# skyhehe123/SA-SSD

Hardware: NVIDIA H100
Metric: KITTI frames/sec (~20k pts, car_cfg voxel grid) (higher is better)
Workload: dtype f32

## Files before the change

include/sassd_b200.h:

```cpp
#ifndef SASSD_B200_H
#define SASSD_B200_H

#include <stddef.h>
#include <stdint.h>

#ifdef __cplusplus
extern "C" {
#endif

typedef void* sassd_stream_t;

enum {
    SASSD_OK = 0,
    SASSD_ERR_ARG = -1,
    SASSD_ERR_LAUNCH = -2,
    SASSD_ERR_WORKSPACE = -3,
    SASSD_ERR_UNSUPPORTED = -4
};

enum {
    SASSD_FLAG_VOXEL_CAP = 1,
    SASSD_FLAG_ROWS_CAP = 2,
    SASSD_FLAG_GUIDED_CAP = 4,
    SASSD_FLAG_NMS_CAP = 8,
// ... 42 lines not shown
int sassd_anchor_mask(const int32_t* coors, const int32_t* d_rows, int rows_cap, int batch, int H, int W,
                      const int32_t* rects, int n_anchors, int threshold, uint8_t* mask,
                      void* ws, size_t ws_bytes, sassd_stream_t stream);

int sassd_hash_build(const int32_t* coors, const int32_t* d_rows, int rows_cap, int batch, int D, int H, int W,
                     int32_t* keys, int32_t* vals, int slots, int32_t* d_status, sassd_stream_t stream);
int sassd_rulebook_subm(const int32_t* coors, const int32_t* d_rows, int rows_cap, int D, int H, int W,
                        const int32_t* keys, const int32_t* vals, int slots, int32_t* nbr, int32_t* tile_mask,
                        sassd_stream_t stream);
size_t sassd_rulebook_conv_workspace_bytes(int batch, int Do, int Ho, int Wo);
int sassd_rulebook_conv_outputs(const int32_t* coors_in, const int32_t* d_rows_in, int rows_cap_in, int batch,
                                int D, int H, int W, int32_t* coors_out, int32_t* d_rows_out, int rows_cap_out,
                                int32_t* d_status, void* ws, size_t ws_bytes, sassd_stream_t stream);
int sassd_rulebook_conv_outputs_hash(const int32_t* coors_in, const int32_t* d_rows_in, int rows_cap_in, int batch,
                                     int D, int H, int W, int32_t* coors_out, int32_t* d_rows_out, int rows_cap_out,
                                     int32_t* keys_out, int32_t* vals_out, int slots_out, int32_t* d_status, void* ws,
                                     size_t ws_bytes, sassd_stream_t stream);
int sassd_rulebook_conv_nbr(const int32_t* coors_out, const int32_t* d_rows_out, int rows_cap_out, int D, int H, int W,
                            const int32_t* keys_in, const int32_t* vals_in, int slots_in, int32_t* nbr,
                            int32_t* tile_mask, sassd_stream_t stream);
int sassd_rulebook_pairs(const int32_t* nbr, const int32_t* d_rows_out, int rows_cap, int32_t* indice_pairs,
                         int32_t* indice_pair_num, sassd_stream_t stream);

enum { SASSD_GCONV_TABLE = 0, SASSD_GCONV_CONV2D = 1, SASSD_GCONV_ROWS = 2 };
enum { SASSD_PREC_FP32 = 0, SASSD_PREC_TF32X3 = 1, SASSD_PREC_F16X3 = 2 };
typedef struct {
    int32_t mode, precision;
    int32_t cin, cout, taps;
    int32_t in_stride, out_stride;
    int32_t rows_cap;
    int32_t batch, H, W;
    int32_t relu;
} sassd_gconv_desc;
int sassd_gconv(const sassd_gconv_desc* host_desc, const float* in, const float* weight, const float* scale,
                const float* shift, const int32_t* nbr, const int32_t* d_rows, float* out, sassd_stream_t stream);

size_t sassd_gconv_pack_bytes(int taps, int cin, int cout, int precision);
int sassd_gconv_pack(const float* weight, int taps, int cin, int cout, int precision, void* packed,
                     sassd_stream_t stream);

typedef struct {
    int32_t batch, H, W;
    int32_t cin, cin_stored;
    int32_t cout, taps, relu;
    int32_t out_f32_stride, out_split_ch;
    int32_t tile_order;
    int32_t n_split;
} sassd_conv2d_desc;
int sassd_conv2d_f16x3(const sassd_conv2d_desc* host_desc, const void* in_split, const void* wpack, const float* scale,
                       const float* shift, float* out_f32, void* out_split, sassd_stream_t stream);
#define SASSD_CONV2D_TILE_H 8
#define SASSD_CONV2D_TILE_W 16
#define SASSD_TILE_DIST_MAX 9
int sassd_conv2d_f16x3_occ(const sassd_conv2d_desc* host_desc, const void* in_split, const void* wpack,
                           const float* scale, const float* shift, float* out_f32, void* out_split,
                           const int32_t* tile_dist, int reach, const float* const_out, int32_t* counters,
                           sassd_stream_t stream);
int sassd_conv2d_f16x3_occ_bg(const sassd_conv2d_desc* host_desc, const void* in_split, const void* wpack,
                              const float* scale, const float* shift, float* out_f32, void* out_split,
                              const int32_t* tile_dist, int reach, const float* const_out, const void* bg_split,
                              const float* bg_f32, int32_t* counters, sassd_stream_t stream);
int sassd_sparse_to_bev_split(const float* feat, const int32_t* coors, const int32_t* d_rows, int rows_cap, int C,
                              int D, int H, int W, int batch, void* bev_split, int32_t* tile_dist,
                              sassd_stream_t stream);

typedef struct {
    int32_t cin, cout, taps;
    int32_t rows_cap, in_rows_cap;
    int32_t relu, out_ch, out_f32_stride;
} sassd_spconv_desc;
size_t sassd_spconv_pack_bytes(int taps, int cin_stored, int cout);
int sassd_spconv_pack(const float* weight, int taps, int cin, int cin_stored, int cout, void* packed,
                      sassd_stream_t stream);
#define SASSD_SPCONV_TILE_ROWS 128
size_t sassd_spconv_workspace_bytes(void);
int sassd_spconv_f16x3(const sassd_spconv_desc* host_desc, const void* in_split, const void* wpack, const float* scale,
                       const float* shift, const int32_t* nbr, const int32_t* tile_mask, const int32_t* d_rows,
                       void* out_split, float* out_f32, void* ws, size_t ws_bytes, int32_t* counters,
                       sassd_stream_t stream);
int sassd_features_to_split(const float* feat, const int32_t* d_rows, int rows_cap, int cin, int cs, void* out_split,
                            sassd_stream_t stream);
int sassd_split_rows_to_bev(const void* feat_split, const int32_t* coors, const int32_t* d_rows, int rows_cap, int C,
                            int D, int H, int W, int batch, void* bev_split, int32_t* tile_dist, sassd_stream_t stream);

int sassd_sparse_to_bev(const float* feat, const int32_t* coors, const int32_t* d_rows, int rows_cap, int C,
                        int D, int H, int W, float* bev, sassd_stream_t stream);

size_t sassd_decode_select_workspace_bytes(int batch, int n_anchors);
int sassd_decode_select(const float* head, int head_stride, int batch, int H, int W, int num_class,
                        const float* anchors, int anchors_per_frame, const uint8_t* mask, int n_anchors, float thr,
                        float* boxes, int32_t* labels, int32_t* index, int32_t* d_k, int k_cap,
                        int32_t* d_status, void* ws, size_t ws_bytes, sassd_stream_t stream);

int sassd_pswarp(const float* feat, int feat_stride, int batch, int H, int W, const float* boxes,
                 const int32_t* d_k, int k_cap, float off_x, float off_y, float spatial_scale,
                 float* scores, sassd_stream_t stream);

size_t sassd_rescore_nms_workspace_bytes(int batch, int k_cap, int nms_cap);
int sassd_rescore_nms(const float* boxes, const float* scores, const int32_t* labels, const int32_t* d_k,
                      int batch, int k_cap, float score_thr, float iou_thr, int nms_cap,
                      float* det, int32_t* d_ndet, int det_cap, int32_t* d_status,
                      void* ws, size_t ws_bytes, sassd_stream_t stream);

#define SASSD_KITTI_META 36
#define SASSD_KITTI_ROW 14
int sassd_kitti_format(const float* det, const int32_t* d_ndet, int batch, int det_cap, const double* meta,
                       double* rows, int32_t* n_out, sassd_stream_t stream);

typedef struct {
    const void* rows;
    int64_t plane_stride;
    int32_t row_stride;
    int32_t channels;
    int32_t split;
    int32_t pad;
} sassd_point_levels;

int sassd_three_nn(const float* mean, const int32_t* coors0, const int32_t* d_rows0, int rows_cap0,
                   const int32_t* coors1, const int32_t* d_rows1, const int32_t* coors2, const int32_t* d_rows2,
                   const int32_t* coors3, const int32_t* d_rows3, int32_t* idx, float* dist2, float* points_mean,
                   sassd_stream_t stream);
int sassd_point_aux_head(const int32_t* idx, const float* dist2, const int32_t* d_rows0, int rows_cap0,
                         const sassd_point_levels* host_levels, const float* w_fc_t, const float* w_out, float* cls,
                         float* reg, sassd_stream_t stream);

#define SASSD_GT_CAP_MAX 256
size_t sassd_loss_workspace_bytes(int batch, int gt_cap);
int sassd_points_in_boxes(const float* points_mean, const int32_t* d_rows, int rows_cap, const float* gt,
                          const int32_t* d_ngt, int batch, int gt_cap, int32_t* labels, float* offsets,
                          int32_t* d_npos, int32_t* d_status, sassd_stream_t stream);
int sassd_assign_rpn(const float* anchors, int anchors_per_frame, const uint8_t* mask, int n_anchors, int num_class,
                     const float* gt, const int32_t* gt_class, const int32_t* gt_label, const int32_t* d_ngt,
                     int batch, int gt_cap, const float* host_pos_thr, const float* host_neg_thr, int32_t* labels,
                     float* targets, float* ious, int32_t* d_npos, int32_t* d_status, void* ws, size_t ws_bytes,
                     sassd_stream_t stream);
int sassd_assign_pswarp(const float* gt, const int32_t* d_ngt, int batch, int gt_cap, const float* boxes, int n_box,
                        const int32_t* d_head, int head_cap, const int32_t* d_k, float pos_thr, float neg_thr,
                        int32_t* labels, float* ious, int32_t* d_npos, int32_t* d_status, void* ws,
                        size_t ws_bytes, sassd_stream_t stream);
int sassd_rpn_loss(const float* head, int head_stride, int batch, int H, int W, int num_class, const float* anchors,
                   int anchors_per_frame, int n_anchors, const int32_t* labels, const float* targets,
                   const int32_t* d_npos, float* out, void* ws, size_t ws_bytes, sassd_stream_t stream);
int sassd_pswarp_loss(const float* scores, const int32_t* labels, int batch, int n_box, const int32_t* d_npos,
                      float* out, void* ws, size_t ws_bytes, sassd_stream_t stream);
int sassd_aux_loss(const float* point_cls, const float* point_reg, const int32_t* labels, const float* offsets,
                   const int32_t* d_rows, int rows_cap, int batch, const int32_t* d_npos, float* out, void* ws,
                   size_t ws_bytes, sassd_stream_t stream);

size_t sassd_nms_workspace_bytes(int n);
int sassd_nms_mask(const float* boxes5, int n, float thr, uint64_t* mask, sassd_stream_t stream);
int sassd_nms_sorted(const float* boxes5, int n, float thr, int64_t* keep, int32_t* d_nkeep,
                     void* ws, size_t ws_bytes, sassd_stream_t stream);
int sassd_boxes_iou_bev(const float* boxes_a, int na, const float* boxes_b, int nb, float* iou, sassd_stream_t stream);

int sassd_rotate_overlap_eval(const float* boxes, const int32_t* box_off, const float* query, const int32_t* query_off,
                              const int64_t* out_off, int nframes, int criterion, int max_pairs_per_frame, float* out,
                              sassd_stream_t stream);
int sassd_kitti_match(int nframes, const double* overlaps, const int64_t* ov_off, const int32_t* gt_off,
                      const int32_t* dt_off, const int32_t* dc_off, const double* gt_alpha, const double* dt_alpha,
                      const double* dt_score, const double* dt_bbox, const double* dc_bbox, const int32_t* ign_gt,
                      const int32_t* ign_dt, int metric, double min_overlap, int compute_aos, int nthresh,
                      const double* thresholds, double* pr, double* tp_scores, int64_t* n_tp_scores);

#ifdef __cplusplus
}
#endif
// ... 2 lines not shown
```

sa-ssd_b200/csrc/spconv_split.cu:

```cuda
#include "tc_common.cuh"

namespace sps {

using namespace tc;

constexpr int BKC = 64;
constexpr int PROD_WARPS = 8;
constexpr int THREADS3 = CONS_THREADS + PROD_WARPS * 32;
constexpr int W_PROD = CONS_THREADS / 32;
constexpr int MAX_CTAS = 148;
constexpr int DEAL_MIN_GAIN = 14;

template <int BN>
struct Cfg3 {
    static constexpr int B_TILE_BYTES = BN * 128;
    static constexpr int STAGE_BYTES = 2 * A_TILE_BYTES + 2 * B_TILE_BYTES;
    static constexpr int STAGES = 4;
    static constexpr int NBR_TILE_BYTES = BM * 27 * 4;
    static constexpr int BAR_BYTES = 768;
    static constexpr int DEAL_INTS = MAX_CTAS + 1 + 33 + 2 + 1;
    static constexpr int SMEM_BYTES = STAGES * STAGE_BYTES + 2 * NBR_TILE_BYTES + 1024 + BAR_BYTES + DEAL_INTS * 4;
};

__device__ __forceinline__ void cp_async16(uint32_t dst, const void* src, uint32_t src_bytes) {
// ... 426 lines not shown

static size_t spconv_parts_bytes() { return (size_t)2 * sps::MAX_CTAS * sps::BM * 64 * sizeof(float); }

extern "C" size_t sassd_spconv_workspace_bytes(void) {
    return spconv_parts_bytes() + (size_t)sps::MAX_CTAS * 2 * sizeof(int32_t);
}

extern "C" int sassd_spconv_f16x3(const sassd_spconv_desc* d, const void* in_split, const void* wpack,
                                  const float* scale, const float* shift, const int32_t* nbr,
                                  const int32_t* tile_mask, const int32_t* d_rows, void* out_split, float* out_f32,
                                  void* ws, size_t ws_bytes, int32_t* counters, sassd_stream_t stream_) {
    if (!d || !in_split || !wpack || (!out_split && !out_f32)) return SASSD_ERR_ARG;
    if (d->cin < 8 || (d->cin & 7) || d->cin > 64 || d->cout < 1 || d->cout > 64 || d->taps < 1 || d->rows_cap < 0)
        return SASSD_ERR_ARG;
    if (d->taps > 1 && !nbr) return SASSD_ERR_ARG;
    if (tile_mask && d->taps > 27) return SASSD_ERR_ARG;
    if (out_split && ((d->out_ch & 7) || d->out_ch < d->cout)) return SASSD_ERR_ARG;
    if (out_f32 && (d->out_f32_stride & 3)) return SASSD_ERR_ARG;
    if (ws && ws_bytes < sassd_spconv_workspace_bytes()) return SASSD_ERR_WORKSPACE;
    if (d->rows_cap == 0) return SASSD_OK;
    sps::Args a;
    a.in = (const __half*)in_split; a.in_plane = (size_t)d->in_rows_cap * d->cin;
    a.wpack = wpack; a.scale = scale; a.shift = shift; a.nbr = nbr; a.tile_mask = tile_mask; a.d_rows = d_rows;
    a.out_split = (__half*)out_split; a.out_plane = (size_t)d->rows_cap * d->out_ch; a.out_f32 = out_f32;
    a.parts = (float*)ws;
    a.arrivals = ws ? (int*)((char*)ws + spconv_parts_bytes()) : nullptr;
    a.counters = counters;
    a.cin = d->cin; a.cout = d->cout; a.taps = d->taps; a.rows_cap = d->rows_cap; a.relu = d->relu;
    a.out_ch = d->out_ch; a.out_f32_stride = d->out_f32_stride;
    const int tiles = sassd_div_up(d->rows_cap, sps::BM), tpg = spconv_tpg(d->cin);
    if (d->taps == 1) return sps::dispatch3<0>(a, tiles, (cudaStream_t)stream_);
    return sps::dispatch3<1>(a, ws ? tiles * ((d->taps + tpg - 1) / tpg) : tiles, (cudaStream_t)stream_);
}

__global__ void features_to_split_kernel(const float* __restrict__ feat, const int* __restrict__ d_rows, int rows_cap,
                                         int cin, int cs, __half* __restrict__ out) {
    const int rows = d_rows ? min(*d_rows, rows_cap) : rows_cap;
    const long long total = (long long)rows * cs;
    const size_t plane = (size_t)rows_cap * cs;
    for (long long i = blockIdx.x * (long long)blockDim.x + threadIdx.x; i < total; i += (long long)gridDim.x * blockDim.x) {
        const int r = (int)(i / cs), c = (int)(i % cs);
        float hi = 0.f, lo = 0.f;
        if (c < cin) tc::split_f16(feat[(size_t)r * cin + c], hi, lo);
        out[i] = __float2half_rn(hi);
        out[i + plane] = __float2half_rn(lo);
    }
}

extern "C" int sassd_features_to_split(const float* feat, const int32_t* d_rows, int rows_cap, int cin, int cs,
                                       void* out_split, sassd_stream_t stream_) {
    if (!feat || !out_split || cin < 1 || cs < cin || (cs & 7)) return SASSD_ERR_ARG;
    if (rows_cap <= 0) return SASSD_OK;
    features_to_split_kernel<<<sassd_grid((long long)rows_cap * cs, 256), 256, 0, (cudaStream_t)stream_>>>(
        feat, d_rows, rows_cap, cin, cs, (__half*)out_split);
    return sassd_check_launch();
}

__global__ void split_rows_to_bev_kernel(const uint4* __restrict__ feat, size_t in_plane16, const int4* __restrict__ coors,
                                         const int* __restrict__ d_rows, int rows_cap, int C8, int D, int H, int W,
                                         size_t out_plane16, uint4* __restrict__ bev, int* __restrict__ tile_dist) {
    const int rows = min(*d_rows, rows_cap);
    const long long total = (long long)rows * C8;
    for (long long i = blockIdx.x * (long long)blockDim.x + threadIdx.x; i < total; i += (long long)gridDim.x * blockDim.x) {
        const int r = (int)(i / C8), q = (int)(i % C8);
        const int4 c = __ldg(&coors[r]);
        const size_t o = (((size_t)c.x * H + c.z) * W + c.w) * (size_t)(D * C8) + (size_t)c.y * C8 + q;
        bev[o] = __ldg(&feat[i]);
        bev[o + out_plane16] = __ldg(&feat[i + in_plane16]);
        if (tile_dist && q == 0) sassd_mark_conv2d_tiles(tile_dist, c.x, c.z, c.w, H, W);
    }
}

extern "C" int sassd_split_rows_to_bev(const void* feat_split, const int32_t* coors, const int32_t* d_rows, int rows_cap,
                                       int C, int D, int H, int W, int batch, void* bev_split, int32_t* tile_dist,
                                       sassd_stream_t stream_) {
    if (!feat_split || !coors || !d_rows || !bev_split || (C & 7) || batch < 1) return SASSD_ERR_ARG;
    if (rows_cap <= 0) return SASSD_OK;
    const size_t in_plane16 = (size_t)rows_cap * C / 8, out_plane16 = (size_t)batch * H * W * D * C / 8;
    split_rows_to_bev_kernel<<<sassd_grid((long long)rows_cap * (C / 8), 256), 256, 0, (cudaStream_t)stream_>>>(
        (const uint4*)feat_split, in_plane16, (const int4*)coors, d_rows, rows_cap, C / 8, D, H, W, out_plane16,
        (uint4*)bev_split, tile_dist);
    return sassd_check_launch();
}
```

sa-ssd_b200/lib.py:

```python
import ctypes
import os

from . import build as _build

c_int, c_float, c_size_t, c_void_p = ctypes.c_int, ctypes.c_float, ctypes.c_size_t, ctypes.c_void_p


class VoxelParams(ctypes.Structure):
    _fields_ = [("voxel_size", c_float * 3), ("range_min", c_float * 3), ("grid", ctypes.c_int32 * 3),
                ("max_points", ctypes.c_int32), ("max_voxels", ctypes.c_int32)]


class Conv2dDesc(ctypes.Structure):
    _fields_ = [(n, ctypes.c_int32) for n in ("batch", "H", "W", "cin", "cin_stored", "cout", "taps", "relu",
                                              "out_f32_stride", "out_split_ch", "tile_order", "n_split")]


class SpconvDesc(ctypes.Structure):
    _fields_ = [(n, ctypes.c_int32) for n in ("cin", "cout", "taps", "rows_cap", "in_rows_cap", "relu", "out_ch",
                                              "out_f32_stride")]


class GConvDesc(ctypes.Structure):
    _fields_ = [(n, ctypes.c_int32) for n in ("mode", "precision", "cin", "cout", "taps", "in_stride", "out_stride",
                                              "rows_cap", "batch", "H", "W", "relu")]


class PointLevels(ctypes.Structure):
    _fields_ = [("rows", c_void_p), ("plane_stride", ctypes.c_int64), ("row_stride", ctypes.c_int32),
                ("channels", ctypes.c_int32), ("split", ctypes.c_int32), ("pad", ctypes.c_int32)]


GCONV_TABLE, GCONV_CONV2D, GCONV_ROWS = 0, 1, 2
PREC_FP32, PREC_TF32X3, PREC_F16X3 = 0, 1, 2
CONV2D_TILE_H, CONV2D_TILE_W = 8, 16
TILE_DIST_MAX = 9
SPCONV_TILE_ROWS = 128
KITTI_META, KITTI_ROW = 36, 14
POINT_LEVEL_CHANNELS = (32, 64, 64)
POINT_FC_IN, POINT_FC_OUT = 160, 64
GT_CAP_MAX = 256

OK = 0
ERRORS = {-1: "SASSD_ERR_ARG", -2: "SASSD_ERR_LAUNCH", -3: "SASSD_ERR_WORKSPACE", -4: "SASSD_ERR_UNSUPPORTED"}
FLAGS = {1: "VOXEL_CAP", 2: "ROWS_CAP", 4: "GUIDED_CAP", 8: "NMS_CAP", 16: "HASH_FULL", 32: "DET_CAP",
         64: "GT_CAP", 128: "GATHER_CAP"}
GATHER_CAP = 128

P = c_void_p
_SIGNATURES = {
    "sassd_version": (c_int, []),
    "sassd_voxelize_workspace_bytes": (c_size_t, [c_int, c_int, c_int]),
    "sassd_voxelize": (c_int, [P, P, c_int, c_int, ctypes.POINTER(VoxelParams), c_int, P, P, P, P, c_int, P, P, P,
                               c_size_t, P]),
    "sassd_voxel_mean": (c_int, [P, P, P, c_int, c_int, P, P]),
    "sassd_frustum_crop_workspace_bytes": (c_size_t, [c_int, c_int]),
    "sassd_frustum_crop": (c_int, [P, P, c_int, c_int, P, P, P, P, c_size_t, P]),
    "sassd_image_fov_crop": (c_int, [P, P, c_int, c_int, P, c_float, P, P, P, c_size_t, P]),
    "sassd_points_in_rbboxes_workspace_bytes": (c_size_t, [c_int, c_int, c_int]),
    "sassd_points_in_rbboxes": (c_int, [P, P, c_int, c_int, P, P, P, c_int, P, P, P, c_int, P, P, c_size_t, P]),
    "sassd_anchor_mask_workspace_bytes": (c_size_t, [c_int, c_int, c_int]),
    "sassd_anchor_mask": (c_int, [P, P, c_int, c_int, c_int, c_int, P, c_int, c_int, P, P, c_size_t, P]),
    "sassd_hash_build": (c_int, [P, P, c_int, c_int, c_int, c_int, c_int, P, P, c_int, P, P]),
    "sassd_rulebook_subm": (c_int, [P, P, c_int, c_int, c_int, c_int, P, P, c_int, P, P, P]),
    "sassd_rulebook_conv_workspace_bytes": (c_size_t, [c_int, c_int, c_int, c_int]),
    "sassd_rulebook_conv_outputs": (c_int, [P, P, c_int, c_int, c_int, c_int, c_int, P, P, c_int, P, P, c_size_t, P]),
    "sassd_set_pdl": (c_int, [c_int]),
    "sassd_rulebook_conv_outputs_hash": (c_int, [P, P, c_int, c_int, c_int, c_int, c_int, P, P, c_int, P, P, c_int, P, P,
                                                 c_size_t, P]),
    "sassd_rulebook_conv_nbr": (c_int, [P, P, c_int, c_int, c_int, c_int, P, P, c_int, P, P, P]),
    "sassd_rulebook_pairs": (c_int, [P, P, c_int, P, P, P]),
    "sassd_gconv": (c_int, [ctypes.POINTER(GConvDesc), P, P, P, P, P, P, P, P]),
    "sassd_gconv_pack_bytes": (c_size_t, [c_int, c_int, c_int, c_int]),
    "sassd_gconv_pack": (c_int, [P, c_int, c_int, c_int, c_int, P, P]),
    "sassd_conv2d_f16x3": (c_int, [ctypes.POINTER(Conv2dDesc), P, P, P, P, P, P, P]),
    "sassd_conv2d_f16x3_occ": (c_int, [ctypes.POINTER(Conv2dDesc), P, P, P, P, P, P, P, c_int, P, P, P]),
    "sassd_conv2d_f16x3_occ_bg": (c_int, [ctypes.POINTER(Conv2dDesc), P, P, P, P, P, P, P, c_int, P, P, P, P, P]),
    "sassd_rotate_overlap_eval": (c_int, [P, P, P, P, P, c_int, c_int, c_int, P, P]),
    "sassd_kitti_match": (c_int, [c_int, P, P, P, P, P, P, P, P, P, P, P, P, c_int, ctypes.c_double, c_int, c_int, P, P,
                                  P, P]),
    "sassd_spconv_pack_bytes": (c_size_t, [c_int, c_int, c_int]),
    "sassd_spconv_pack": (c_int, [P, c_int, c_int, c_int, c_int, P, P]),
    "sassd_spconv_workspace_bytes": (c_size_t, []),
    "sassd_spconv_f16x3": (c_int, [ctypes.POINTER(SpconvDesc), P, P, P, P, P, P, P, P, P, P, c_size_t, P, P]),
    "sassd_features_to_split": (c_int, [P, P, c_int, c_int, c_int, P, P]),
    "sassd_split_rows_to_bev": (c_int, [P, P, P, c_int, c_int, c_int, c_int, c_int, c_int, P, P, P]),
    "sassd_sparse_to_bev_split": (c_int, [P, P, P, c_int, c_int, c_int, c_int, c_int, c_int, P, P, P]),
    "sassd_sparse_to_bev": (c_int, [P, P, P, c_int, c_int, c_int, c_int, c_int, P, P]),
    "sassd_decode_select_workspace_bytes": (c_size_t, [c_int, c_int]),
    "sassd_decode_select": (c_int, [P, c_int, c_int, c_int, c_int, c_int, P, c_int, P, c_int, c_float, P, P, P, P, c_int, P,
                                    P, c_size_t, P]),
    "sassd_pswarp": (c_int, [P, c_int, c_int, c_int, c_int, P, P, c_int, c_float, c_float, c_float, P, P]),
    "sassd_rescore_nms_workspace_bytes": (c_size_t, [c_int, c_int, c_int]),
    "sassd_rescore_nms": (c_int, [P, P, P, P, c_int, c_int, c_float, c_float, c_int, P, P, c_int, P, P, c_size_t, P]),
    "sassd_kitti_format": (c_int, [P, P, c_int, c_int, P, P, P, P]),
    "sassd_three_nn": (c_int, [P, P, P, c_int, P, P, P, P, P, P, P, P, P, P]),
    "sassd_point_aux_head": (c_int, [P, P, P, c_int, ctypes.POINTER(PointLevels), P, P, P, P, P]),
    "sassd_nms_workspace_bytes": (c_size_t, [c_int]),
    "sassd_nms_mask": (c_int, [P, c_int, c_float, P, P]),
    "sassd_nms_sorted": (c_int, [P, c_int, c_float, P, P, P, c_size_t, P]),
    "sassd_boxes_iou_bev": (c_int, [P, c_int, P, c_int, P, P]),
    "sassd_loss_workspace_bytes": (c_size_t, [c_int, c_int]),
    "sassd_points_in_boxes": (c_int, [P, P, c_int, P, P, c_int, c_int, P, P, P, P, P]),
    "sassd_assign_rpn": (c_int, [P, c_int, P, c_int, c_int, P, P, P, P, c_int, c_int, P, P, P, P, P, P, P, P, c_size_t,
                                 P]),
    "sassd_assign_pswarp": (c_int, [P, P, c_int, c_int, P, c_int, P, c_int, P, c_float, c_float, P, P, P, P, P, c_size_t,
                                    P]),
    "sassd_rpn_loss": (c_int, [P, c_int, c_int, c_int, c_int, c_int, P, c_int, c_int, P, P, P, P, P, c_size_t, P]),
    "sassd_pswarp_loss": (c_int, [P, P, c_int, c_int, P, P, P, c_size_t, P]),
    "sassd_aux_loss": (c_int, [P, P, P, P, P, c_int, c_int, P, P, P, c_size_t, P]),
}

_LIB = None


class SassdError(RuntimeError):
    pass


def exported_symbols():
    return sorted(_SIGNATURES)


def load(build_if_missing=True):
    global _LIB
    if _LIB is not None:
        return _LIB
    path = _build.LIB
    if not os.path.exists(path):
        if not build_if_missing:
            raise SassdError("libsassd_b200.so not built: run `python -m sassd_b200.build`")
        path = _build.build()
    lib = ctypes.CDLL(path)
    for name, (res, args) in _SIGNATURES.items():
        try:
            fn = getattr(lib, name)
        except AttributeError as e:
            raise SassdError("libsassd_b200.so lacks symbol %s (stale build?)" % name) from e
        fn.restype = res
        fn.argtypes = args
    _LIB = lib
    return lib


def check(rc, what):
    if rc != OK:
        raise SassdError("%s failed: %s (%d)" % (what, ERRORS.get(rc, "unknown"), rc))


def decode_flags(word):
    return [name for bit, name in FLAGS.items() if word & bit]


def raise_on_status(word):
    word = int(word)
    if word:
        raise SassdError("capacity overflow on device: %s" % decode_flags(word))
```

sa-ssd_b200/necks.py:

```python
import torch
from torch import nn

from . import ops, spconv
from .spconv import fold_bn, _versions


def single_conv(in_channels, out_channels, indice_key=None):
    return spconv.SparseSequential(
        spconv.SubMConv3d(in_channels, out_channels, 1, bias=False, indice_key=indice_key),
        nn.BatchNorm1d(out_channels, eps=1e-3, momentum=0.01),
        nn.ReLU(),
    )


def _subm_block(n, in_channels, out_channels, indice_key):
    layers = []
    for i in range(n):
        layers += [spconv.SubMConv3d(in_channels if i == 0 else out_channels, out_channels, 3, bias=False,
                                     indice_key=indice_key),
                   nn.BatchNorm1d(out_channels, eps=1e-3, momentum=0.01), nn.ReLU()]
    return spconv.SparseSequential(*layers)


def double_conv(in_channels, out_channels, indice_key=None):
# ... 86 lines not shown
def pack_conv2d_weight(w, dc_order=None):
    cout, cin, kh, kw = w.shape
    p = w.detach().permute(2, 3, 1, 0).reshape(kh * kw, cin, cout)
    if dc_order is not None:
        C, D = dc_order
        p = p.reshape(kh * kw, C, D, cout).permute(0, 2, 1, 3).reshape(kh * kw, cin, cout)
    return p.contiguous().float()


def conv2d_nhwc(x, weight_packed, scale, shift, relu, cout, precision=ops.PREC_FP32, out=None, split_out=False):
    if isinstance(x, ops.SplitMap):
        sp, f32 = ops.conv2d_split(x, weight_packed, scale, shift, relu, cout, out_split=split_out,
                                   out_f32=not split_out)
        return sp if split_out else f32
    B, H, W, cin = x.shape
    taps = weight_packed.shape[0]
    stride = (cout + 3) // 4 * 4
    if out is None:
        out = torch.empty((B, H, W, stride), dtype=torch.float32, device=x.device)
        if stride != cout:
            out.zero_()
    ops.gconv(x.view(-1, cin), weight_packed, scale, shift, out.view(-1, out.shape[-1]), mode=ops.GCONV_CONV2D,
              taps=taps, cin=cin, cout=cout, relu=relu, rows_cap=B * H * W, batch=B, H=H, W=W, precision=precision)
    return out


class BEVNet(nn.Module):

    def __init__(self, in_features, num_filters=256):
        super().__init__()
        for i in range(8):
            k = 1 if i == 7 else 3
            setattr(self, "conv%d" % i, nn.Conv2d(in_features if i == 0 else num_filters, num_filters, k,
                                                  padding=k // 2, bias=False))
            setattr(self, "bn%d" % i, nn.BatchNorm2d(num_filters, eps=1e-3, momentum=0.01))
        self.num_filters = num_filters
        self.precision = ops.DEFAULT_PRECISION
        self._packed = {}

    def _weights(self, i, dc_order):
        conv = getattr(self, "conv%d" % i)
        key = (i, dc_order)
        ver = _versions(conv.weight)
        c = self._packed.get(key)
        if c is None or c[0] != ver:
            c = (ver, pack_conv2d_weight(conv.weight, dc_order))
            self._packed[key] = c
        return c[1]

    def forward_nhwc(self, x, dc_order=None):
        if self.training:
            raise NotImplementedError("sassd_b200 is inference-only: call .eval()")
        split = isinstance(x, ops.SplitMap)
        for i in range(7):
            scale, shift = fold_bn(getattr(self, "bn%d" % i))
            x = conv2d_nhwc(x, self._weights(i, dc_order if i == 0 else None), scale, shift, True, self.num_filters,
                            self.precision, split_out=split)
        conv6 = x
        scale, shift = fold_bn(self.bn7)
        x = conv2d_nhwc(x, self._weights(7, None), scale, shift, True, self.num_filters, self.precision,
                        split_out=split)
        return x, conv6

    def forward(self, x):
        ops.require_cuda()
        xh = x.permute(0, 2, 3, 1).contiguous()
        y, c6 = self.forward_nhwc(xh)
        return y.permute(0, 3, 1, 2), c6.permute(0, 3, 1, 2)


class SpMiddleFHD(nn.Module):

    def __init__(self, output_shape, num_input_features=4, num_hidden_features=128):
        super().__init__()
        self.sparse_shape = list(output_shape)
        self.backbone = VxNet(num_input_features)
        self.fcn = BEVNet(in_features=num_hidden_features, num_filters=256)
        self.point_fc = nn.Linear(160, 64, bias=False)
        self.point_cls = nn.Linear(64, 1, bias=False)
        self.point_reg = nn.Linear(64, 3, bias=False)
        self.row_cap_factor = 4
        self.dense_tma = True
        self.overlap_rulebooks = True
        self._side = None
        self._point_packed = None

    def _point_weights(self):
        ver = _versions(self.point_fc.weight, self.point_cls.weight, self.point_reg.weight)
        c = self._point_packed
        if c is None or c[0] != ver:
            with torch.no_grad():
                fc_t = self.point_fc.weight.detach().t().contiguous().float()
                out = torch.cat([self.point_cls.weight.detach(), self.point_reg.weight.detach()], 0).contiguous().float()
            c = self._point_packed = (ver, fc_t, out)
        return c[1], c[2]

    def point_head(self, mean, coors, d_rows, middle):
        levels = [(m._indices, m.d_rows) for m in middle]
        idx, dist2, pm = ops.three_nn(mean, coors, d_rows, levels, points_mean=True)
        feats = []
        for m, ch in zip(middle, ops._lib.POINT_LEVEL_CHANNELS):
            if m._features is not None:
                feats.append(ops.point_level(feat=m._features, channels=ch))
            else:
                feats.append(ops.point_level(split=m._split, channels=ch))
        fc_t, w_out = self._point_weights()
        cls, reg = ops.point_aux_head(idx, dist2, d_rows, feats, fc_t, w_out)
        return dict(points_mean=pm, point_cls=cls, point_reg=reg, idx=idx, dist2=dist2, middle=middle)

    def build_aux_target(self, nxyz, gt_boxes3d, enlarge=1.0):
        labels, offsets, _ = self._aux_targets(nxyz, gt_boxes3d, enlarge)
        return labels.to(torch.uint8), offsets

    def _aux_targets(self, nxyz, gt_boxes3d, enlarge=1.0):
        from .single_stage_heads import stage_gt
        ops.require_cuda()
        dev = nxyz.device if nxyz.is_cuda else torch.device("cuda")
        boxes = []
        for g in gt_boxes3d:
            g = torch.as_tensor(g, dtype=torch.float32).reshape(-1, 7).clone()
            g[:, 3:6] *= enlarge
            boxes.append(g)
        gt, _, _, d_ngt = stage_gt(boxes, None, None, dev)
        pm = nxyz.to(dev).float().contiguous()
        n = pm.shape[0]
        if n == 0:
            return torch.zeros(0, dtype=torch.int32, device=dev), torch.zeros((0, 3), device=dev), None
        status = torch.zeros((1,), dtype=torch.int32, device=dev)
        d_rows = torch.tensor([n], dtype=torch.int32, device=dev)
        labels, offsets, d_npos = ops.points_in_boxes(pm, d_rows, gt, d_ngt, status)
        ops._lib.raise_on_status(status)
        return labels, offsets, (d_rows, d_npos)

    def aux_loss(self, points, point_cls, point_reg, gt_bboxes):
        labels, offsets, rows = self._aux_targets(points, gt_bboxes)
        dev = labels.device
        out = torch.zeros((2,), dtype=torch.float32, device=dev)
        if rows is not None:
            d_rows, d_npos = rows
            ops.aux_loss(point_cls.reshape(-1).float().contiguous(), point_reg.float().contiguous(), labels, offsets,
                         d_rows, len(gt_bboxes), d_npos, out)
        return dict(aux_loss_cls=out[0:1], aux_loss_reg=out[1:2])

    def set_precision(self, precision, sparse=None):
        self.backbone.set_precision(precision if sparse is None else sparse)
        self.fcn.precision = precision

    def forward_nhwc(self, voxel_features, coors, batch_size, d_rows=None, status=None, point_outputs=False):
        if self.training:
            raise NotImplementedError("sassd_b200 is inference-only: call .eval()")
        x = spconv.SparseConvTensor(voxel_features, coors, self.sparse_shape, batch_size, d_rows=d_rows, status=status)
        x.row_cap_factor = self.row_cap_factor
        x0_mean, x0_coors, rows0 = x._features, x._indices, x.d_rows
        if self.overlap_rulebooks:
            if self._side is None:
                self._side = torch.cuda.Stream(device=x.device)
                self._side2 = torch.cuda.Stream(device=x.device)
            self.backbone.prebuild_rulebooks(x, self._side, self._side2)
        x, middle = self.backbone(x)
        if self.overlap_rulebooks:
            torch.cuda.current_stream().wait_stream(self._side)
        pts = None
        if point_outputs:
            pts = self.point_head(x0_mean, x0_coors, rows0, middle)
        C = x._channels
        D, H, W = x.spatial_shape
        if self.fcn.precision == ops.PREC_F16X3 and self.dense_tma:
            if x._split is not None and x._split.shape[2] == C:
                bev = ops.split_rows_to_bev(x._split, x._indices, x.d_rows, C, D, H, W, batch_size)
            else:
                bev = ops.sparse_to_bev_split(x.features_cap(), x._indices, x.d_rows, C, D, H, W, batch_size)
        else:
            feats = x.features_cap()
            bev = torch.zeros((batch_size, H, W, D * C), dtype=torch.float32, device=feats.device)
            ops.sparse_to_bev(feats, x._indices, x.d_rows, C, D, H, W, bev)
        y, conv6 = self.fcn.forward_nhwc(bev, dc_order=(C, D))
        if point_outputs:
            return y, conv6, x, pts
        return y, conv6, x

    def forward(self, voxel_features, coors, batch_size, is_test=False, d_rows=None, status=None):
        if not is_test and self.training:
            raise NotImplementedError("the auxiliary training branch (cmn.py:44-100) is out of scope: call .eval()")
        out = self.forward_nhwc(voxel_features, coors, batch_size, d_rows, status, point_outputs=not is_test)
        y, conv6 = out[0], out[1]
        if isinstance(y, ops.SplitMap):
            y, conv6 = y.float(), conv6.float()
        y, conv6 = y.permute(0, 3, 1, 2), conv6.permute(0, 3, 1, 2)
        if is_test:
            return y, conv6
        pts = out[3]
        n = voxel_features.shape[0] if d_rows is None else int(d_rows.reshape(-1)[0].item())
        return y, conv6, (pts["points_mean"][:n], pts["point_cls"][:n].unsqueeze(1), pts["point_reg"][:n])
```

sa-ssd_b200/ops.py:

```python
import collections
import ctypes
import os
import math

import numpy as np
import torch

from . import lib as _lib
from .lib import Conv2dDesc, SpconvDesc
from .lib import (GCONV_CONV2D, GCONV_ROWS, GCONV_TABLE, PREC_F16X3, PREC_FP32, PREC_TF32X3, GConvDesc, VoxelParams,
                  check)

NMS_CAP = 4096
DEFAULT_PRECISION = PREC_F16X3


def _L():
    return _lib.load()


def _stream():
    return ctypes.c_void_p(torch.cuda.current_stream().cuda_stream)


def _ptr(t):
    if t is None:
        return ctypes.c_void_p(0)
    assert t.is_cuda and t.is_contiguous(), "sassd ops need contiguous CUDA tensors"
    return ctypes.c_void_p(t.data_ptr())


def require_cuda():
    if not torch.cuda.is_available():
        raise _lib.SassdError("sassd_b200 needs a CUDA device (sm_90a); there is no CPU fallback")


def next_pow2(n):
    return 1 << max(1, int(math.ceil(math.log2(max(2, n)))))


_KERNELS = {"sassd_voxelize": 4, "sassd_voxel_mean": 1, "sassd_frustum_crop": 1, "sassd_image_fov_crop": 1, "sassd_points_in_rbboxes": 1, "sassd_anchor_mask": 4, "sassd_hash_build": 1,
            "sassd_rulebook_subm": 1, "sassd_rulebook_conv_outputs": 2, "sassd_rulebook_conv_outputs_hash": 2, "sassd_rulebook_conv_nbr": 1,
            "sassd_rulebook_pairs": 1, "sassd_gconv": 1, "sassd_gconv_pack": 1, "sassd_spconv_pack": 1, "sassd_rotate_overlap_eval": 1, "sassd_conv2d_f16x3": 1, "sassd_conv2d_f16x3_occ": 1, "sassd_conv2d_f16x3_occ_bg": 1, "sassd_spconv_f16x3": 1, "sassd_features_to_split": 1, "sassd_split_rows_to_bev": 1, "sassd_sparse_to_bev_split": 1, "sassd_sparse_to_bev": 1, "sassd_decode_select": 2,
            "sassd_pswarp": 1, "sassd_rescore_nms": 3, "sassd_kitti_format": 1, "sassd_three_nn": 1, "sassd_point_aux_head": 1, "sassd_nms_mask": 1, "sassd_nms_sorted": 2,
            "sassd_boxes_iou_bev": 1, "sassd_points_in_boxes": 2, "sassd_assign_rpn": 3, "sassd_assign_pswarp": 3,
            "sassd_rpn_loss": 2, "sassd_pswarp_loss": 2, "sassd_aux_loss": 2}
LAUNCHES = 0
PROFILE = None


def _call(name, label, *args):
    global LAUNCHES
    LAUNCHES += _KERNELS[name]
    fn = getattr(_L(), name)
    if PROFILE is None:
        check(fn(*args), name)
        return
    e0 = torch.cuda.Event(enable_timing=True)
    e1 = torch.cuda.Event(enable_timing=True)
    e0.record()
    check(fn(*args), name)
    e1.record()
    PROFILE.append((name, label, e0, e1))


class Workspace:

    def __init__(self):
        self._bufs = {}

    def get(self, key, nbytes, device, zeroed=False):
        buf = self._bufs.get(key)
        if buf is None or buf.numel() < nbytes or buf.device != device:
            buf = (torch.zeros if zeroed else torch.empty)(max(int(nbytes), 256), dtype=torch.uint8, device=device)
            self._bufs[key] = buf
        return buf


_WS = Workspace()


def make_voxel_params(voxel_size, pc_range, max_points, max_voxels):
    vs = np.asarray(voxel_size, np.float32)
    rg = np.asarray(pc_range, np.float32)
    grid = np.round((rg[3:] - rg[:3]) / vs).astype(np.int64)
    p = VoxelParams()
    for j in range(3):
        p.voxel_size[j] = float(vs[j]); p.range_min[j] = float(rg[j]); p.grid[j] = int(grid[j])
    p.max_points = int(max_points); p.max_voxels = int(max_voxels)
    return p, grid


def voxelize(points, pt_off, batch, params, rows_cap, slots_per_frame, status, want_mean=True, ws=None):
    dev = points.device
    n_cap = points.shape[0]
    voxels = torch.empty((rows_cap, params.max_points, 4), dtype=torch.float32, device=dev)
    coors = torch.empty((rows_cap, 4), dtype=torch.int32, device=dev)
    num = torch.empty((rows_cap,), dtype=torch.int32, device=dev)
    mean = torch.empty((rows_cap, 4), dtype=torch.float32, device=dev) if want_mean else None
    frame_rows = torch.empty((batch + 1,), dtype=torch.int32, device=dev)
    nbytes = _L().sassd_voxelize_workspace_bytes(n_cap, batch, slots_per_frame)
    w = (ws or _WS).get("voxelize", nbytes, dev)
    _call("sassd_voxelize", None, _ptr(points), _ptr(pt_off), n_cap, batch, ctypes.byref(params), slots_per_frame,
                              _ptr(voxels), _ptr(coors), _ptr(num), _ptr(mean), rows_cap, _ptr(frame_rows),
                              _ptr(status), _ptr(w), w.numel(), _stream())
    return voxels, coors, num, mean, frame_rows


def frustum_crop(points, pt_off, batch, planes, ws=None):
    dev = points.device
    n_cap = points.shape[0]
    assert planes.dtype == torch.float64 and tuple(planes.shape) == (batch, 6, 4), "planes must be float64 [batch,6,4]"
    out = torch.empty_like(points)
    off = torch.empty((batch + 1,), dtype=torch.int32, device=dev)
    nbytes = _L().sassd_frustum_crop_workspace_bytes(n_cap, batch)
    w = (ws or _WS).get("frustum", nbytes, dev)
    _call("sassd_frustum_crop", None, _ptr(points), _ptr(pt_off), n_cap, batch, _ptr(planes), _ptr(out), _ptr(off),
          _ptr(w), w.numel(), _stream())
    return out, off


IMAGE_FOV_CLIP_X = 0.1


def image_fov_crop(points, pt_off, batch, meta, clip_x=IMAGE_FOV_CLIP_X, ws=None):
    dev = points.device
# ... 495 lines not shown
    dist = _tile_dist(batch, H, W, feat.device)
    _call("sassd_sparse_to_bev_split", None, _ptr(feat), _ptr(coors), _ptr(d_rows), feat.shape[0], C, D, H, W, batch,
          _ptr(planes), _ptr(dist), _stream())
    return SplitMap(planes, D * C, dist)


def conv2d_split(x, weight, scale, shift, relu, cout, out_split=True, out_f32=False):
    B, H, W, cin = x.shape
    taps = weight.shape[0]
    wp = tc_pack_cached(weight, PREC_F16X3)
    d = Conv2dDesc()
    d.batch, d.H, d.W, d.cin, d.cin_stored = B, H, W, cin, x.planes.shape[-1]
    d.cout, d.taps, d.relu = cout, taps, 1 if relu else 0
    d.tile_order = CONV2D_TILE_ORDER
    d.n_split = 0
    osp = of = None
    if out_split:
        cs = (cout + 63) // 64 * 64
        alloc = torch.empty if cs == cout else torch.zeros
        osp = alloc((2, B, H, W, cs), dtype=torch.float16, device=x.device)
        d.out_split_ch = cs
    if out_f32:
        stride = (cout + 3) // 4 * 4
        of = torch.empty((B, H, W, stride), dtype=torch.float32, device=x.device)
        d.out_f32_stride = stride
    label = "conv2d_tma[taps=%d %d->%d]" % (taps, cin, cout)
    dist = x.tile_dist if TILE_OCCUPANCY else None
    reach, cvec, bg_sp, bg_f = 0, None, None, None
    if dist is not None:
        reach = x.reach + (1 if taps == 9 else 0)
        if not tile_skipping_valid(H, W, reach):
            dist = None
    if dist is not None:
        cvec = conv_constant(x.const, cin, weight, scale, shift, relu, cout)
        bg = conv_background(x, weight, scale, shift, relu, cout, out_split, out_f32)
        if bg is not None:
            bg_sp, bg_f = bg
    _call("sassd_conv2d_f16x3_occ_bg", label, ctypes.byref(d), _ptr(x.planes), _ptr(wp), _ptr(scale), _ptr(shift),
          _ptr(of), _ptr(osp), _ptr(dist), reach, _ptr(cvec), _ptr(bg_sp.planes if bg_sp is not None else None),
          _ptr(bg_f), _ptr(CONV2D_COUNTERS.get(label) if CONV2D_COUNTERS is not None else None), _stream())
    return (SplitMap(osp, cout, dist, reach, cvec, bg_sp) if osp is not None else None), of


def features_to_split(feat, d_rows=None):
    cap, C = feat.shape
    cs = (C + 7) // 8 * 8
    out = torch.empty((2, cap, cs), dtype=torch.float16, device=feat.device)
    _call("sassd_features_to_split", None, _ptr(feat), _ptr(d_rows), cap, C, cs, _ptr(out), _stream())
    return out


def split_rows_float(planes, channels):
    return (planes[0].float() + planes[1].float() * (1.0 / 2048.0))[:, :channels].contiguous()


SPCONV_COUNTERS = None
SPCONV_TAP_SKIP = os.environ.get("SASSD_SPS_SKIP", "1") != "0"
SPCONV_TAP_SPLIT = os.environ.get("SASSD_SPS_SPLIT", "1") != "0"


def spconv_split(planes, weight, scale, shift, relu, cout, rows_cap, nbr=None, d_rows=None, want_f32=False,
                 tile_mask=None, ws=None):
    taps = weight.shape[0]
    wp = spconv_pack_cached(weight, planes.shape[2])
    d = SpconvDesc()
    d.cin, d.cout, d.taps = planes.shape[2], cout, taps
    d.rows_cap, d.in_rows_cap, d.relu = rows_cap, planes.shape[1], 1 if relu else 0
    d.out_ch = (cout + 7) // 8 * 8
    out = torch.empty((2, rows_cap, d.out_ch), dtype=torch.float16, device=planes.device)
    of = None
    if want_f32:
        d.out_f32_stride = (cout + 3) // 4 * 4
        of = torch.empty((rows_cap, d.out_f32_stride), dtype=torch.float32, device=planes.device)
    label = "spconv_split[taps=%d %d->%d]" % (taps, weight.shape[1], cout)
    w = None
    if SPCONV_TAP_SPLIT and taps > 1:
        w = (ws or _WS).get("spconv_split", _L().sassd_spconv_workspace_bytes(), planes.device, zeroed=True)
    _call("sassd_spconv_f16x3", label, ctypes.byref(d), _ptr(planes), _ptr(wp), _ptr(scale), _ptr(shift), _ptr(nbr),
          _ptr(tile_mask if SPCONV_TAP_SKIP else None), _ptr(d_rows), _ptr(out), _ptr(of), _ptr(w),
          0 if w is None else w.numel(), _ptr(SPCONV_COUNTERS), _stream())
    return out, of


def split_rows_to_bev(planes, coors, d_rows, C, D, H, W, batch):
    bev = torch.zeros((2, batch, H, W, D * C), dtype=torch.float16, device=planes.device)
    dist = _tile_dist(batch, H, W, planes.device)
    _call("sassd_split_rows_to_bev", None, _ptr(planes), _ptr(coors), _ptr(d_rows), planes.shape[1], C, D, H, W, batch,
          _ptr(bev), _ptr(dist), _stream())
    return SplitMap(bev, D * C, dist)
```

Baseline: 801.6.

## Prepare BEV buffer and tile distances on side stream, zeroing only read tiles

Adds a bev_prepare path that builds the tile-distance map from the final rulebook's output coordinates on a side stream while the sparse backbone runs. The BEV split buffer is then cleared only for tiles near occupied ones, instead of a full torch.zeros on the critical path. split_rows_to_bev reuses the prepared buffer and skips its own tile marking. The risk is that uncleared tiles hold garbage, which is safe only if downstream conv2d tile skipping never reads them. It also adds cross-stream ordering that must be correct, relying on the existing wait on the side stream.

```diff
diff --git a/include/sassd_b200.h b/include/sassd_b200.h
--- a/include/sassd_b200.h
+++ b/include/sassd_b200.h
@@ -148,6 +148,9 @@
                             sassd_stream_t stream);
 int sassd_split_rows_to_bev(const void* feat_split, const int32_t* coors, const int32_t* d_rows, int rows_cap, int C,
                             int D, int H, int W, int batch, void* bev_split, int32_t* tile_dist, sassd_stream_t stream);
+#define SASSD_TILE_FAR (1 << 20)
+int sassd_bev_prepare(const int32_t* coors, const int32_t* d_rows, int rows_cap, int channels, int H, int W, int batch,
+                      int reach, void* bev_split, int32_t* tile_dist, sassd_stream_t stream);
 
 int sassd_sparse_to_bev(const float* feat, const int32_t* coors, const int32_t* d_rows, int rows_cap, int C,
                         int D, int H, int W, float* bev, sassd_stream_t stream);
diff --git a/sa-ssd_b200/csrc/spconv_split.cu b/sa-ssd_b200/csrc/spconv_split.cu
--- a/sa-ssd_b200/csrc/spconv_split.cu
+++ b/sa-ssd_b200/csrc/spconv_split.cu
@@ -532,3 +532,60 @@
         (uint4*)bev_split, tile_dist);
     return sassd_check_launch();
 }
+
+__global__ void bev_dist_init_kernel(int* __restrict__ tile_dist, int ntiles) {
+    const int i = blockIdx.x * blockDim.x + threadIdx.x;
+    if (i < ntiles) tile_dist[i] = SASSD_TILE_FAR;
+}
+
+__global__ void bev_mark_kernel(const int4* __restrict__ coors, const int* __restrict__ d_rows, int rows_cap, int H,
+                                int W, int* __restrict__ tile_dist) {
+    const int rows = min(*d_rows, rows_cap);
+    for (int r = blockIdx.x * blockDim.x + threadIdx.x; r < rows; r += gridDim.x * blockDim.x) {
+        const int4 c = __ldg(&coors[r]);
+        sassd_mark_conv2d_tiles(tile_dist, c.x, c.z, c.w, H, W);
+    }
+}
+
+__global__ void __launch_bounds__(256) bev_zero_read_tiles_kernel(const int* __restrict__ tile_dist, int H, int W,
+                                                                  int vpp, int reach, size_t plane16,
+                                                                  uint4* __restrict__ bev) {
+    const int tiles_x = (W + SASSD_CONV2D_TILE_W - 1) / SASSD_CONV2D_TILE_W;
+    const int tiles_y = (H + SASSD_CONV2D_TILE_H - 1) / SASSD_CONV2D_TILE_H;
+    const int b = blockIdx.x / (tiles_y * tiles_x), ty = (blockIdx.x / tiles_x) % tiles_y, tx = blockIdx.x % tiles_x;
+    __shared__ int s_read;
+    if (threadIdx.x < 32) {
+        const int ny = ty + (int)threadIdx.x / 3 - 1, nx = tx + (int)threadIdx.x % 3 - 1;
+        const bool read = threadIdx.x < 9 && ny >= 0 && ny < tiles_y && nx >= 0 && nx < tiles_x &&
+                          tile_dist[(b * tiles_y + ny) * tiles_x + nx] <= reach;
+        const unsigned m = __ballot_sync(0xffffffffu, read);
+        if (threadIdx.x == 0) s_read = m != 0u;
+    }
+    __syncthreads();
+    if (!s_read) return;
+    const int y0 = ty * SASSD_CONV2D_TILE_H, x0 = tx * SASSD_CONV2D_TILE_W;
+    const int rows = min(SASSD_CONV2D_TILE_H, H - y0), run = min(SASSD_CONV2D_TILE_W, W - x0) * vpp;
+    const uint4 z = make_uint4(0u, 0u, 0u, 0u);
+    for (int i = threadIdx.x; i < rows * run; i += blockDim.x) {
+        const size_t o = (((size_t)b * H + y0 + i / run) * W + x0) * vpp + i % run;
+        bev[o] = z;
+        bev[o + plane16] = z;
+    }
+}
+
+extern "C" int sassd_bev_prepare(const int32_t* coors, const int32_t* d_rows, int rows_cap, int channels, int H, int W,
+                                 int batch, int reach, void* bev_split, int32_t* tile_dist, sassd_stream_t stream_) {
+    if (!coors || !d_rows || !bev_split || !tile_dist || (channels & 7) || batch < 1 || H < 1 || W < 1 || reach < 0)
+        return SASSD_ERR_ARG;
+    const cudaStream_t stream = (cudaStream_t)stream_;
+    const int ntiles = batch * ((H + SASSD_CONV2D_TILE_H - 1) / SASSD_CONV2D_TILE_H) *
+                       ((W + SASSD_CONV2D_TILE_W - 1) / SASSD_CONV2D_TILE_W);
+    bev_dist_init_kernel<<<sassd_div_up(ntiles, 256), 256, 0, stream>>>(tile_dist, ntiles);
+    if (rows_cap > 0)
+        bev_mark_kernel<<<sassd_grid(rows_cap, 256), 256, 0, stream>>>((const int4*)coors, d_rows, rows_cap, H, W,
+                                                                       tile_dist);
+    const size_t plane16 = (size_t)batch * H * W * channels / 8;
+    bev_zero_read_tiles_kernel<<<ntiles, 256, 0, stream>>>(tile_dist, H, W, channels / 8, reach, plane16,
+                                                           (uint4*)bev_split);
+    return sassd_check_launch();
+}
diff --git a/sa-ssd_b200/lib.py b/sa-ssd_b200/lib.py
--- a/sa-ssd_b200/lib.py
+++ b/sa-ssd_b200/lib.py
@@ -86,6 +86,7 @@
     "sassd_features_to_split": (c_int, [P, P, c_int, c_int, c_int, P, P]),
     "sassd_split_rows_to_bev": (c_int, [P, P, P, c_int, c_int, c_int, c_int, c_int, c_int, P, P, P]),
     "sassd_sparse_to_bev_split": (c_int, [P, P, P, c_int, c_int, c_int, c_int, c_int, c_int, P, P, P]),
+    "sassd_bev_prepare": (c_int, [P, P, c_int, c_int, c_int, c_int, c_int, c_int, P, P, P]),
     "sassd_sparse_to_bev": (c_int, [P, P, P, c_int, c_int, c_int, c_int, c_int, P, P]),
     "sassd_decode_select_workspace_bytes": (c_size_t, [c_int, c_int]),
     "sassd_decode_select": (c_int, [P, c_int, c_int, c_int, c_int, c_int, P, c_int, P, c_int, c_float, P, P, P, P, c_int, P,
diff --git a/sa-ssd_b200/necks.py b/sa-ssd_b200/necks.py
--- a/sa-ssd_b200/necks.py
+++ b/sa-ssd_b200/necks.py
@@ -192,6 +192,7 @@
         self.row_cap_factor = 4
         self.dense_tma = True
         self.overlap_rulebooks = True
+        self.bev_prepare = True
         self._side = None
         self._point_packed = None
 
@@ -262,11 +263,19 @@
         x = spconv.SparseConvTensor(voxel_features, coors, self.sparse_shape, batch_size, d_rows=d_rows, status=status)
         x.row_cap_factor = self.row_cap_factor
         x0_mean, x0_coors, rows0 = x._features, x._indices, x.d_rows
+        split_bev = self.fcn.precision == ops.PREC_F16X3 and self.dense_tma
+        prep = None
         if self.overlap_rulebooks:
             if self._side is None:
                 self._side = torch.cuda.Stream(device=x.device)
                 self._side2 = torch.cuda.Stream(device=x.device)
             self.backbone.prebuild_rulebooks(x, self._side, self._side2)
+            if split_bev and self.bev_prepare:
+                rb = x.indice_dict["down2"]
+                D3, H3, W3 = rb.shape_out
+                prep = (rb.coors_out, ops.bev_prepare(rb.coors_out, rb.d_rows_out,
+                                                      self.backbone.extra_conv[0].out_channels, D3, H3, W3,
+                                                      batch_size, self._side))
         x, middle = self.backbone(x)
         if self.overlap_rulebooks:
             torch.cuda.current_stream().wait_stream(self._side)
@@ -275,9 +284,11 @@
             pts = self.point_head(x0_mean, x0_coors, rows0, middle)
         C = x._channels
         D, H, W = x.spatial_shape
-        if self.fcn.precision == ops.PREC_F16X3 and self.dense_tma:
+        if split_bev:
             if x._split is not None and x._split.shape[2] == C:
-                bev = ops.split_rows_to_bev(x._split, x._indices, x.d_rows, C, D, H, W, batch_size)
+                use = prep is not None and prep[1] is not None and prep[0] is x._indices
+                bev = ops.split_rows_to_bev(x._split, x._indices, x.d_rows, C, D, H, W, batch_size,
+                                            prepared=prep[1] if use else None)
             else:
                 bev = ops.sparse_to_bev_split(x.features_cap(), x._indices, x.d_rows, C, D, H, W, batch_size)
         else:
diff --git a/sa-ssd_b200/ops.py b/sa-ssd_b200/ops.py
--- a/sa-ssd_b200/ops.py
+++ b/sa-ssd_b200/ops.py
@@ -41,7 +41,7 @@
 
 _KERNELS = {"sassd_voxelize": 4, "sassd_voxel_mean": 1, "sassd_frustum_crop": 1, "sassd_image_fov_crop": 1, "sassd_points_in_rbboxes": 1, "sassd_anchor_mask": 4, "sassd_hash_build": 1,
             "sassd_rulebook_subm": 1, "sassd_rulebook_conv_outputs": 2, "sassd_rulebook_conv_outputs_hash": 2, "sassd_rulebook_conv_nbr": 1,
-            "sassd_rulebook_pairs": 1, "sassd_gconv": 1, "sassd_gconv_pack": 1, "sassd_spconv_pack": 1, "sassd_rotate_overlap_eval": 1, "sassd_conv2d_f16x3": 1, "sassd_conv2d_f16x3_occ": 1, "sassd_conv2d_f16x3_occ_bg": 1, "sassd_spconv_f16x3": 1, "sassd_features_to_split": 1, "sassd_split_rows_to_bev": 1, "sassd_sparse_to_bev_split": 1, "sassd_sparse_to_bev": 1, "sassd_decode_select": 2,
+            "sassd_rulebook_pairs": 1, "sassd_gconv": 1, "sassd_gconv_pack": 1, "sassd_spconv_pack": 1, "sassd_rotate_overlap_eval": 1, "sassd_conv2d_f16x3": 1, "sassd_conv2d_f16x3_occ": 1, "sassd_conv2d_f16x3_occ_bg": 1, "sassd_spconv_f16x3": 1, "sassd_features_to_split": 1, "sassd_split_rows_to_bev": 1, "sassd_sparse_to_bev_split": 1, "sassd_bev_prepare": 3, "sassd_sparse_to_bev": 1, "sassd_decode_select": 2,
             "sassd_pswarp": 1, "sassd_rescore_nms": 3, "sassd_kitti_format": 1, "sassd_three_nn": 1, "sassd_point_aux_head": 1, "sassd_nms_mask": 1, "sassd_nms_sorted": 2,
             "sassd_boxes_iou_bev": 1, "sassd_points_in_boxes": 2, "sassd_assign_rpn": 3, "sassd_assign_pswarp": 3,
             "sassd_rpn_loss": 2, "sassd_pswarp_loss": 2, "sassd_aux_loss": 2}
@@ -703,9 +703,24 @@
     return out, of
 
 
-def split_rows_to_bev(planes, coors, d_rows, C, D, H, W, batch):
-    bev = torch.zeros((2, batch, H, W, D * C), dtype=torch.float16, device=planes.device)
-    dist = _tile_dist(batch, H, W, planes.device)
+def split_rows_to_bev(planes, coors, d_rows, C, D, H, W, batch, prepared=None):
+    if prepared is None:
+        bev = torch.zeros((2, batch, H, W, D * C), dtype=torch.float16, device=planes.device)
+        dist = mark = _tile_dist(batch, H, W, planes.device)
+    else:
+        (bev, dist), mark = prepared, None
     _call("sassd_split_rows_to_bev", None, _ptr(planes), _ptr(coors), _ptr(d_rows), planes.shape[1], C, D, H, W, batch,
-          _ptr(bev), _ptr(dist), _stream())
+          _ptr(bev), _ptr(mark), _stream())
     return SplitMap(bev, D * C, dist)
+
+
+def bev_prepare(coors, d_rows, C, D, H, W, batch, stream):
+    if not TILE_OCCUPANCY or not tile_skipping_valid(H, W, 1):
+        return None
+    th, tw = _lib.CONV2D_TILE_H, _lib.CONV2D_TILE_W
+    bev = torch.empty((2, batch, H, W, D * C), dtype=torch.float16, device=coors.device)
+    dist = torch.empty((batch * ((H + th - 1) // th) * ((W + tw - 1) // tw),), dtype=torch.int32, device=coors.device)
+    stream.wait_stream(torch.cuda.current_stream())
+    _call("sassd_bev_prepare", None, _ptr(coors), _ptr(d_rows), coors.shape[0], D * C, H, W, batch, 1, _ptr(bev),
+          _ptr(dist), ctypes.c_void_p(stream.cuda_stream))
+    return bev, dist
```

Result: no change. 820.1, median of 6 (+2.3%).
